# rpp0/gr-lora

Measured on AMD Instinct MI355X. Metric: IQ Msamples/s demodulated, higher is better.
Workload: dtype f32

## Files before the change

### gr_lora_amd/build.py

```python
from __future__ import annotations

import os
import shutil
import subprocess

_HERE = os.path.dirname(os.path.abspath(__file__))
CSRC = os.path.join(_HERE, "csrc")
LIB = os.path.join(_HERE, "liblora_hip.so")
SOURCES = ["lora_kernels.hip", "lora_runtime.cpp", "lora_channelizer.hip", "lora_filterbank.hip", "lora_iq_unpack.hip", "lora_gateway.cpp", "lora_frame_check.cpp", "lora_tx.hip"]
DEPS = SOURCES + ["lora_device.h", "lora_stitch.hpp", "lora_walker2.inc.hip", "lora_walker3.inc.hip", "lora_team_demod.inc.hip", "lora_wave_demod.inc.hip", "lora_wave_decim.inc.hip", "lora_detect.inc.hip", "lora_strict_sync.inc.hip", "lora_strict_resolve_lds.inc", "whitening_data.inc", "lora_mux_dev.h", "lora_iq.h", "lora_frame_check.h",
                  os.path.join("..", "..", "include", "lora_hip.h"), os.path.join("..", "..", "include", "lora_hip_channelizer.h"),
                  os.path.join("..", "..", "include", "lora_hip_filterbank.h"), os.path.join("..", "..", "include", "lora_hip_gateway.h"),
                  os.path.join("..", "..", "include", "lora_hip_tx.h")]


CODEGEN_FLAGS = ["-mllvm", "-greedy-reverse-local-assignment"]


def hipcc_path() -> str:
    return shutil.which("hipcc") or "/opt/rocm/bin/hipcc"


def stale() -> bool:
    if not os.path.exists(LIB):
        return True
    t = os.path.getmtime(LIB)
    return any(os.path.getmtime(os.path.join(CSRC, d)) > t for d in DEPS)


def build_library(force: bool = False, verbose: bool = False) -> str:
    if not force and not stale():
        return LIB
    cmd = [hipcc_path(), "--offload-arch=gfx950", "-O3", "-std=c++17", "-fPIC", "-shared", "-x", "hip",
           "-Wall", "-Wno-unused-function"] + CODEGEN_FLAGS + os.environ.get("LORA_HIP_EXTRA_FLAGS", "").split() + ["-I", CSRC, "-o", LIB] + [os.path.join(CSRC, s) for s in SOURCES]
    if verbose:
        cmd.insert(1, "-Rpass-analysis=kernel-resource-usage")
    subprocess.check_call(cmd)
    return LIB


if __name__ == "__main__":
    import sys
    print(build_library(force=True, verbose="-v" in sys.argv))
# ... 1 lines not shown
```

### gr_lora_amd/csrc/lora_device.h

```cpp
#pragma once
#include <stdint.h>

#if !defined(__HIPCC__) && !defined(HIP_INCLUDE_HIP_HIP_RUNTIME_H)
struct float2 { float x, y; };
#endif

namespace lora_hip {

constexpr int kWG = 256;
constexpr int kMaxBinsPerThread = 16;
constexpr int kMaxFrame = 3 + 255 + 2;
constexpr int kMaxCodewords = 640;

enum DecState : int32_t { kDetect = 0, kSync, kFindSfd, kPause, kDecodeHeader, kDecodePayload, kStop };

enum AttemptStatus : uint32_t {
    kAttemptNone = 0,
    kAttemptFrame = 1,
    kAttemptLostSync = 2,
    kAttemptOutOfData = 3,
    kAttemptAtHeader = 4,
    kAttemptAtSfd = 5,
    kAttemptHeaderOnly = 6
};
struct SkippedPayload {
    uint8_t  phdr[3];
    uint8_t  n_left;
    uint8_t  left[8];
    int32_t  payload_symbols;
};
constexpr float kSfdIllVar = 1.0f / 4096.0f;
constexpr int kMaxSfdRec = 12;

struct DevParams {
    uint32_t sf, nbins, nbins_hdr, sps, decim, log_nbins, delay_after_sync;
    uint32_t implicit, reduced_rate, enable_fine_sync, demod_mode;
    uint32_t ctor_cr, ctor_crc;
    uint32_t use_fast;
// ... 69 lines not shown
    int64_t  tail_final_pos;
    uint32_t tail_valid, tail_first_rec, tail_n_attempts, tail_final_cr, tail_npush, tail_stop_reason, tail_pad, tail_rsv;
    float    tail_push_tail[4];
    uint32_t ctl[4];
    uint32_t dbg[6];
};

struct StepRec {
    int32_t  state, consumed;
    int64_t  pos;
    int32_t  bin, fine;
    float    value;
    uint32_t stream;
    uint32_t cycles;
    uint32_t pad;
};

struct LaunchCfg {
    const float2 *iq;
    const Job *jobs;
    JobResult *results;
    AttemptRec *recs;
    uint32_t recs_per_job;
    float *scratch;
    StepRec *trace;
    uint32_t trace_cap;
    uint32_t n_jobs;
    uint32_t *balance;
    uint32_t skip_payload;
};
constexpr uint32_t kBalanceCus = 2048;
constexpr uint32_t kBalanceWords = 3u * kBalanceCus;

struct EnvStream {
    uint64_t off;
    uint32_t first_block;
    uint32_t n_blocks;
};
int launch_envelope(const float2 *iq, const EnvStream *streams , uint32_t n_streams, uint32_t sps,
                    float *d_E, unsigned long long *d_bitmap , void *stream);

int launch_walker(const DevParams &p, const LaunchCfg &c, void *stream);
const char *walker_kernel_name(const DevParams &p);
struct DemodAlt { int32_t *shift; uint32_t *bins; int32_t *fine; int64_t max_start; };
int launch_demod_symbols(const DevParams &p, const float2 *iq, const int64_t *d_offsets, uint32_t n,
                         int demod, uint32_t *d_bins, int32_t *d_fine, float *scratch, void *stream, const DemodAlt *alt = nullptr);
int launch_detect_windows(const DevParams &p, const float2 *iq, const int64_t *d_offsets, uint32_t n, void *d_out , void *stream);
constexpr int kPayloadHyp = 4;
struct PayloadDesc {
    uint32_t n_walk;
    uint32_t n_hyp;
    int32_t  hyp_shift[kPayloadHyp];
    int32_t  hyp_base[kPayloadHyp];
    uint32_t hyp_from[kPayloadHyp];
    uint32_t hyp_to[kPayloadHyp];
    int64_t  room;
    SkippedPayload sk;
};
enum PayloadWalk : uint32_t { kWalkComplete = 0, kWalkOutOfData = 1, kWalkNeedShift = 2 };
struct PayloadOut {
    uint32_t result;
    uint32_t at;
    int32_t  shift;
    uint32_t frame_len;
    uint8_t  frame[kMaxFrame + 4];
};
int launch_payload_chain(const DevParams &p, const uint32_t *d_bins, const int32_t *d_fine, const DemodAlt &alt, const PayloadDesc *descs, PayloadOut *outs, uint32_t n_packets, void *stream);
bool walker_has_skip_variant(const DevParams &p);
int launch_ref_ifreq(const float2 *x, uint32_t n, float *d_arg, float *d_ifreq, void *stream);
int launch_cfo(const DevParams &p, const float2 *iq, const int64_t *d_offsets, uint32_t n, int mode, float *d_out, void *stream);
bool walker3_covers(uint32_t sf);
uint32_t w3_tw_entries(uint32_t sf);
void build_w3_tables(uint32_t sf, float2 *tw, float2 *ctab );
// ... 13 lines not shown
```

### gr_lora_amd/csrc/lora_kernels.hip

```cpp

#include <hip/hip_runtime.h>
#include <math.h>
#include <stdio.h>
#include <atomic>
#include <cstdlib>
#include <stdint.h>
#include <type_traits>

#include "lora_device.h"
#include "whitening_data.inc"

namespace lora_hip {

__constant__ unsigned char c_whiten_cr56[LORA_WHITEN_CR56_LEN];
__constant__ unsigned char c_whiten_cr78[LORA_WHITEN_CR78_LEN];
__constant__ unsigned char c_h84_decode[256];
static std::atomic<bool> g_consts_ready[16];

static unsigned char h_hamming_encode(unsigned v)
{
    const unsigned b0 = v & 1u, b1 = (v >> 1) & 1u, b2 = (v >> 2) & 1u, b3 = (v >> 3) & 1u;
    const unsigned p1 = b1 ^ b2 ^ b3, p2 = b0 ^ b1 ^ b2, p3 = b0 ^ b1 ^ b3, p4 = b0 ^ b2 ^ b3;
    return (unsigned char)(p1 | (b0 << 1) | (b1 << 2) | (b2 << 3) | (p2 << 4) | (b3 << 5) | (p3 << 6) | (p4 << 7));
}
// ... 773 lines not shown

        if (end_step(st_in, consumed, step_bin, fine, step_val, t_start)) break;
    }

    if (in_attempt && n_att < C.recs_per_job && t0) {
        AttemptRec &r = recs[n_att];
        r.status = (stop_reason == 3u) ? kAttemptAtHeader : kAttemptOutOfData;
        r.start_pos = att_start; r.trig_pos = att_trig; r.hdr_pos = att_hdr; r.end_pos = pos;
        r.npush = npush;
        for (int i = 0; i < 4; i++) r.push_tail[i] = push_tail[i];
        r.cr_prev = att_cr_prev; r.hdr_ambig = att_ambig; r.n_symbols = n_sym; r.frame_len = 0; r.n_sfd = 0;
    }
    if (t0) {
        JobResult &jr = C.results[jid];
        jr.final_pos = in_attempt ? att_start : pos;
        jr.n_attempts = n_att + (in_attempt ? 1u : 0u);
        jr.final_cr = cr;
        jr.npush = in_attempt ? 0u : npush;
        for (int i = 0; i < 4; i++) jr.push_tail[i] = push_tail[i];
        jr.stop_reason = stop_reason;
        jr.n_steps = n_steps < C.trace_cap ? n_steps : C.trace_cap;
        jr.pad = in_attempt ? 1u : 0u;
        for (int i = 0; i < 6; i++) { jr.cyc[i] = 0; jr.rounds[i] = 0; }
        jr.tail_valid = 0;
    }
}

__global__ __launch_bounds__(kWG) void walker_kernel(DevParams P, LaunchCfg C) { walker_body<2>(P, C); }
__global__ __launch_bounds__(kWG) void walker_kernel_f1(DevParams P, LaunchCfg C) { walker_body<1>(P, C); }
__global__ __launch_bounds__(kWG) void walker_kernel_f0(DevParams P, LaunchCfg C) { walker_body<0>(P, C); }

#include "lora_wave_demod.inc.hip"
#include "lora_wave_decim.inc.hip"
#include "lora_walker2.inc.hip"
#include "lora_walker3.inc.hip"
#include "lora_team_demod.inc.hip"

__global__ __launch_bounds__(kWG) void demod_symbols_kernel(DevParams P, const float2 *iq, const int64_t *offsets,
                                                            uint32_t n, int demod, uint32_t *bins, float *scratch)
{
    extern __shared__ __attribute__((aligned(16))) unsigned char smem[];
    float2 *work = reinterpret_cast<float2 *>(smem);
    float *fl = reinterpret_cast<float *>(smem);
    Shared &sh = *reinterpret_cast<Shared *>(smem + P.lds_work_bytes);
    for (uint32_t s = blockIdx.x; s < n; s += gridDim.x) {
        const float2 *x = iq + offsets[s];
        uint32_t b;
        if (demod == 0) {
            float *f1 = P.ifreq_in_lds_1 ? fl : scratch + (size_t)blockIdx.x * 2u * P.sps;
            compute_ifreq(x, P.sps, f1);
            b = gradient_idx_from_ifreq(P, f1, sh.red);
        } else {
            b = get_shift_fft(P, x, work, sh.red);
        }
        if (threadIdx.x == 0) bins[s] = b;
        __syncthreads();
    }
}

constexpr uint32_t kPayloadMaxWalk = 1024;
__global__ __launch_bounds__(64) void payload_chain_kernel(DevParams P, const uint32_t *__restrict__ bins, const int32_t *__restrict__ fine, DemodAlt alt,
                                                           const PayloadDesc *__restrict__ descs, PayloadOut *__restrict__ outs, uint32_t n_packets)
{
    __shared__ Shared sh;
    __shared__ PayloadDesc d;
    __shared__ uint32_t src[kPayloadMaxWalk];
// ... 231 lines not shown
    if (ensure_constants() != 0) return -1;
    if (c.skip_payload && !walker_has_skip_variant(p)) return -1;
    const WalkerKernel k = pick_for_launch(p, c.n_jobs, c.skip_payload != 0);
    if (k.lds > 64u * 1024u) {
        static thread_local const void *last_fn = nullptr;
        static thread_local uint32_t last_lds = 0;
        static thread_local int last_dev = -1;
        int dev = 0;
        (void)hipGetDevice(&dev);
        if (last_fn != (const void *)k.fn || last_lds < k.lds || last_dev != dev) {
            if (hipFuncSetAttribute((const void *)k.fn, hipFuncAttributeMaxDynamicSharedMemorySize, (int)k.lds) != hipSuccess) return -1;
            last_fn = (const void *)k.fn; last_lds = k.lds; last_dev = dev;
        }
    }
    hipLaunchKernelGGL(k.fn, dim3(c.n_jobs), dim3(k.threads), k.lds, (hipStream_t)stream, p, c);
    return hipGetLastError() == hipSuccess ? 0 : -1;
}

uint32_t walker_resident_slots(const DevParams &p)
{
    return slots_of(pick_walker(p, w3_has_half(p) && w3_half_policy() != 0));
}
uint32_t walker_resident_slots_full(const DevParams &p)
{
    if (use_fast_kernel(p) || use_fast_decim(p)) {
        int dev = 0, cus = 0;
        if (hipGetDevice(&dev) != hipSuccess || hipDeviceGetAttribute(&cus, hipDeviceAttributeMultiprocessorCount, dev) != hipSuccess || cus <= 0) cus = 256;
        const uint32_t s = slots_of(pick_walker(p));
        return s > (uint32_t)cus ? (uint32_t)cus : 0u;
    }
    return (w3_has_half(p) && w3_half_policy() < 0) ? slots_of(pick_walker(p, false)) : 0u;
}

constexpr int kEnvLines = 4;
constexpr uint32_t kEnvTableMax = 64;
struct EnvTable { EnvStream s[kEnvTableMax]; };

__global__ __launch_bounds__(256) void envelope_kernel(const float2 *iq, EnvTable T, uint32_t sps, float *E)
{
    const EnvStream s = T.s[blockIdx.y];
    const uint32_t b = (blockIdx.x * 256u + threadIdx.x) >> 3, li = threadIdx.x & 7u;
    const bool live = b < s.n_blocks;
    float e = 0.0f;
    if (live) {
        const float4 *x = reinterpret_cast<const float4 *>(iq + ((s.off + (uint64_t)b * sps) & ~1ull)) + li;
        const uint32_t stride = sps >> 3;
        float4 v[kEnvLines];
#pragma unroll
        for (int l = 0; l < kEnvLines; l++) v[l] = x[(uint32_t)l * stride];
#pragma unroll
        for (int l = 0; l < kEnvLines; l++) e += v[l].x * v[l].x + v[l].y * v[l].y + v[l].z * v[l].z + v[l].w * v[l].w;
    }
    e += __shfl_xor(e, 1); e += __shfl_xor(e, 2); e += __shfl_xor(e, 4);
    if (live && li == 0) E[s.first_block + b] = e;
}

constexpr int kEnvReach = 8;

__global__ __launch_bounds__(256) void edges_kernel(EnvTable T, const float *E, unsigned long long *bitmap)
{
    const EnvStream s = T.s[blockIdx.y];
    const uint32_t b = blockIdx.x * 256u + threadIdx.x;
    bool edge = false;
    if (b >= 1u && b < s.n_blocks) {
        const float *Es = E + s.first_block;
        float m1 = 0.0f, m0 = 0.0f;
#pragma unroll
        for (int d = -kEnvReach - 1; d <= kEnvReach; d++) {
            const int64_t q = (int64_t)b + d;
            const float v = (q >= 0 && q < (int64_t)s.n_blocks) ? Es[q] : 0.0f;
            if (d >= -kEnvReach) m1 = fmaxf(m1, v);
            if (d < kEnvReach) m0 = fmaxf(m0, v);
        }
        edge = Es[b] < 0.5f * m1 && !(Es[b - 1u] < 0.5f * m0);
    }
    const unsigned long long word = __ballot(edge);
    if ((threadIdx.x & 63u) == 0u && b < s.n_blocks) bitmap[(s.first_block + b) >> 6] = word;
}

int launch_envelope(const float2 *iq, const EnvStream *streams , uint32_t n_streams, uint32_t sps, float *d_E,
                    unsigned long long *d_bitmap, void *stream)
{
    if (n_streams == 0 || sps < 128u) return -1;
    for (uint32_t s0 = 0; s0 < n_streams; s0 += kEnvTableMax) {
        const uint32_t n = n_streams - s0 < kEnvTableMax ? n_streams - s0 : kEnvTableMax;
        EnvTable T{};
        uint32_t most = 0;
        for (uint32_t i = 0; i < n; i++) { T.s[i] = streams[s0 + i]; most = most > T.s[i].n_blocks ? most : T.s[i].n_blocks; }
        if (most == 0) continue;
        hipLaunchKernelGGL(envelope_kernel, dim3((most + 31u) / 32u, n), dim3(256), 0, (hipStream_t)stream, iq, T, sps, d_E);
        hipLaunchKernelGGL(edges_kernel, dim3((most + 255u) / 256u, n), dim3(256), 0, (hipStream_t)stream, T, (const float *)d_E, d_bitmap);
    }
    return hipGetLastError() == hipSuccess ? 0 : -1;
}

__global__ __launch_bounds__(256) void cfo_kernel(DevParams P, const float2 *__restrict__ iq, const int64_t *__restrict__ offsets, uint32_t n, int mode,
                                                  float *__restrict__ out)
{
    __shared__ double dred[256];
    const uint32_t sps = P.sps;
    for (uint32_t s = blockIdx.x; s < n; s += gridDim.x) {
        const float2 *x = iq + offsets[s];
        auto dechirped = [&](uint32_t i) {
            const float2 a = x[i], b = P.down[i];
            return make_float2(a.x * b.x - a.y * b.y, a.x * b.y + a.y * b.x);
        };
        if (mode == 0) {
            if (threadIdx.x == 0) out[s] = (float)((double)ifreq_pair(dechirped(256u), dechirped(257u)) / (2.0 * M_PI) * (double)P.samples_per_second);
            continue;
        }
        double acc = 0.0;
        for (uint32_t i = threadIdx.x; i + 1u < sps; i += blockDim.x) acc += (double)ifreq_pair(dechirped(i), dechirped(i + 1u));
        dred[threadIdx.x] = acc;
        __syncthreads();
        for (uint32_t h = 128u; h >= 1u; h >>= 1) {
            if (threadIdx.x < h) dred[threadIdx.x] += dred[threadIdx.x + h];
            __syncthreads();
        }
        if (threadIdx.x == 0) out[s] = (float)(dred[0] / (double)(sps - 1u) / (2.0 * M_PI) * (double)P.samples_per_second);
        __syncthreads();
    }
}

__global__ void ref_ifreq_kernel(const float2 *__restrict__ x, uint32_t n, float *__restrict__ arg_out, float *__restrict__ ifreq_out)
// ... 144 lines not shown
```

### gr_lora_amd/csrc/lora_runtime.cpp

```cpp

#include <hip/hip_runtime.h>

#include <algorithm>
#include <cmath>
#include <cstddef>
#include <cstdarg>
#include <cstdio>
#include <cstdlib>
#include <cstring>
#include <chrono>
#include <deque>
#include <new>
#include <string>
#include <vector>

#include "../../include/lora_hip.h"
#include "lora_device.h"
#include "lora_stitch.hpp"
#include "lora_mux_dev.h"
#include "lora_iq.h"

using namespace lora_hip;

namespace {
// ... 100 lines not shown
    size_t n_up_ifreq_v = 0;
    DevBuf<Job> d_jobs;
    DevBuf<JobResult> d_results;
    DevBuf<AttemptRec> d_recs;
    DevBuf<float> d_scratch;
    DevBuf<StepRec> d_trace;
    DevBuf<float2> d_staging;
    DevBuf<int64_t> d_offsets;
    DevBuf<uint32_t> d_bins;
    RunOut run_out[2];
    std::vector<JobResult> h_results;
    std::vector<AttemptRec> h_recs;
    std::vector<StepRec> h_trace;
    hipEvent_t ev0 = nullptr, ev1 = nullptr, ev_done = nullptr;
    hipEvent_t ev_pre0 = nullptr, ev_pre1 = nullptr, ev_dep = nullptr;
    hipStream_t pre_stream = nullptr;
    struct Pending { uint32_t nj = 0, recs_per_job = 0, eager = 0, trace_cap = 0; bool direct = true, open = false; hipStream_t st = nullptr;
                     std::chrono::steady_clock::time_point hp0, hp1; } pending;
    PassCtx pass;
    std::vector<StreamDesc> pass_streams;
    const float2 *pass_iq = nullptr;
    hipStream_t pass_st = nullptr;
    bool pass_open = false, iq_ready = false;
    bool pre_issued = false;
    const float2 *pre_iq = nullptr;
    uint64_t pre_sig = 0;
    uint32_t pre_ns = 0;
    std::chrono::steady_clock::time_point pre_hq0;
    FrameQueue frames;
    PinnedBuf<Job> p_jobs;
    PinnedBuf<JobResult> p_res;
    PinnedBuf<AttemptRec> p_recs;
    DevBuf<uint32_t> d_balance;
    DevBuf<float> d_env_E;
    DevBuf<unsigned long long> d_env_buf;
    PinnedBuf<EnvStream> p_env_streams;
    PinnedBuf<unsigned long long> p_env_buf;
    float envelope_ms = 0.0f;
    std::vector<lora_hip_step_t> trace;
    lora_hip_timing_t timing{};
    std::string err;
    ChunkPipe pipe;
    struct HostFeed {
        PinnedBuf<float2> stage[2];
        hipEvent_t stage_ev[2] = {nullptr, nullptr};
        bool stage_busy[2] = {false, false};
        int stage_i = 0;
        DevBuf<uint32_t> d_raw;
        std::vector<std::pair<uintptr_t, uintptr_t>> pinned;
        std::vector<std::pair<uintptr_t, uintptr_t>> refused;
    } feed;
    const char *last_kernel = nullptr;
    uint32_t last_kernel_jobs = 0;
    uint32_t resident_slots = 0;
    uint32_t resident_slots_alt = ~0u;
    uint32_t eager_recs = 4;
    uint32_t last_plan_burst = 0, last_plan_segments = 0;
    int decoupled_policy = -1;
    bool launch_skip = false;
    uint32_t dec_backoff = 0;
    uint32_t last_payload_packets = 0, last_payload_rerun = 0, last_payload_symbols = 0, last_payload_moved = 0, last_payload_rounds = 0;
    float last_payload_ms = 0.0f;
    PinnedBuf<int64_t> p_pay_off;
    PinnedBuf<PayloadDesc> p_pay_desc;
    PinnedBuf<PayloadOut> p_pay_out;
    DevBuf<int32_t> d_fine, d_alt_shift, d_alt_fine;
    DevBuf<uint32_t> d_alt_bins;
// ... 219 lines not shown
        HIP_TRY(h, h->d_recs.reserve((size_t)nj * recs_per_job));
    }
    const bool need_scratch = !h->P.ifreq_in_lds_2;
    if (need_scratch) HIP_TRY(h, h->d_scratch.reserve((size_t)nj * 2u * h->P.sps));
    if (trace_cap) HIP_TRY(h, h->d_trace.reserve((size_t)nj * trace_cap));
    static const bool direct = getenv("LORA_HIP_STAGED") == nullptr;
    const uint32_t eager = direct ? recs_per_job : std::min(std::max(h->eager_recs, 2u), recs_per_job);
    HIP_TRY(h, h->p_jobs.reserve(nj));
    HIP_TRY(h, h->p_res.reserve(nj));
    HIP_TRY(h, h->p_recs.reserve((size_t)nj * eager));
    std::memcpy(h->p_jobs.p, jobs.data(), nj * sizeof(Job));
    if (!direct) HIP_TRY(h, hipMemcpyAsync(h->d_jobs.p, h->p_jobs.p, nj * sizeof(Job), hipMemcpyHostToDevice, st));
    LaunchCfg c{};
    c.iq = d_iq; c.recs_per_job = recs_per_job;
    c.jobs = direct ? h->p_jobs.p : h->d_jobs.p; c.results = direct ? h->p_res.p : h->d_results.p; c.recs = direct ? h->p_recs.p : h->d_recs.p;
    c.scratch = need_scratch ? h->d_scratch.p : nullptr;
    c.trace = trace_cap ? h->d_trace.p : nullptr; c.trace_cap = trace_cap; c.n_jobs = nj;
    static const bool no_balance = getenv("LORA_HIP_NO_BALANCE") != nullptr;
    if (!h->d_balance.p && !no_balance) {
        HIP_TRY(h, h->d_balance.reserve(kBalanceWords));
        HIP_TRY(h, hipMemsetAsync(h->d_balance.p, 0, kBalanceWords * sizeof(uint32_t), st));
    }
    c.balance = no_balance ? nullptr : h->d_balance.p;
    c.skip_payload = h->launch_skip ? 1u : 0u;
    HIP_TRY(h, hipEventRecord(h->ev0, st));
    if (nj >= h->last_kernel_jobs) { h->last_kernel = walker_kernel_name_for(h->P, nj, h->launch_skip); h->last_kernel_jobs = nj; }
    if (launch_walker(h->P, c, st) != 0) return fail(h, LORA_HIP_ERR_HIP, "walker launch failed: %s", hipGetErrorString(hipGetLastError()));
    HIP_TRY(h, hipEventRecord(h->ev1, st));
    if (!direct) {
        HIP_TRY(h, hipMemcpyAsync(h->p_res.p, h->d_results.p, nj * sizeof(JobResult), hipMemcpyDeviceToHost, st));
        HIP_TRY(h, hipMemcpy2DAsync(h->p_recs.p, eager * sizeof(AttemptRec), h->d_recs.p, recs_per_job * sizeof(AttemptRec), eager * sizeof(AttemptRec), nj,
                                    hipMemcpyDeviceToHost, st));
    }
    HIP_TRY(h, hipEventRecord(h->ev_done, st));
    h->pending.eager = eager; h->pending.direct = direct; h->pending.open = true;
    h->pending.hp1 = std::chrono::steady_clock::now();
    return LORA_HIP_OK;
}

lora_hip_status run_jobs_end(lora_hip_decoder *h, RunOut &out)
{
    if (!h->pending.open) return LORA_HIP_OK;
    h->pending.open = false;
    const uint32_t nj = h->pending.nj, recs_per_job = h->pending.recs_per_job, eager = h->pending.eager, trace_cap = h->pending.trace_cap;
    const hipStream_t st = h->pending.st;
    const auto hp0 = h->pending.hp0, hp1 = h->pending.hp1;
    const Job *jobs = h->p_jobs.p;
    HIP_TRY(h, hipEventSynchronize(h->ev_done));
    const auto hp2 = std::chrono::steady_clock::now();
    std::memcpy(out.res.data(), h->p_res.p, nj * sizeof(JobResult));
    static const bool dbg_stats = getenv("LORA_HIP_DEBUG") != nullptr;
    if (dbg_stats && h->P.use_fast) {
        double cyc[6] = {0}, rnd[6] = {0};
        for (uint32_t j = 0; j < nj; j++) for (int i = 0; i < 6; i++) { cyc[i] += 64.0 * out.res[j].cyc[i]; rnd[i] += out.res[j].rounds[i]; }
        fprintf(stderr, "[lora_hip] per-job avg kcycles (rounds): DETECT %.0f (%.1f) SYNC %.0f (%.1f) SFD %.0f (%.1f) PAUSE %.0f (%.1f) HDR %.0f (%.1f) PAYLOAD %.0f (%.1f)\n",
                cyc[0] / nj / 1e3, rnd[0] / nj, cyc[1] / nj / 1e3, rnd[1] / nj, cyc[2] / nj / 1e3, rnd[2] / nj, cyc[3] / nj / 1e3, rnd[3] / nj, cyc[4] / nj / 1e3, rnd[4] / nj, cyc[5] / nj / 1e3, rnd[5] / nj);
        {
            double na = 0, nt = 0, ntv = 0; uint32_t sr[4] = {0, 0, 0, 0}, tsr[4] = {0, 0, 0, 0}, tpad = 0;
            for (uint32_t j = 0; j < nj; j++) {
                const JobResult &r = out.res[j];
                na += r.n_attempts; sr[r.stop_reason & 3u]++;
                if (r.tail_valid) { ntv++; nt += r.tail_n_attempts; tsr[r.tail_stop_reason & 3u]++; tpad += r.tail_pad; }
            }
            fprintf(stderr, "[lora_hip] attempts/job %.2f, stop reasons %u/%u/%u/%u; tails %.0f (attempts/tail %.2f, stop reasons %u/%u/%u/%u, pending %u)\n", na / nj, sr[0], sr[1],
                    sr[2], sr[3], ntv, ntv ? nt / ntv : 0.0, tsr[0], tsr[1], tsr[2], tsr[3], tpad);
        }
        double ctl[4] = {0};
        for (uint32_t j = 0; j < nj; j++) for (int i = 0; i < 4; i++) ctl[i] += 64.0 * out.res[j].ctl[i];
        fprintf(stderr, "[lora_hip] control per job, kcycles: copy-in %.0f loop %.0f plan %.0f copy-out %.0f (walker3: demodulation %.0f, replay %.0f of the decode rounds; with LORA_W3_REPLAY_STATS=2 copy-in and symbol loop in the 3rd / 4th figure)\n", ctl[0] / nj / 1e3, ctl[1] / nj / 1e3, ctl[2] / nj / 1e3, ctl[3] / nj / 1e3, ctl[0] / nj / 1e3, ctl[1] / nj / 1e3);
        std::vector<double> tot(nj);
        for (uint32_t j = 0; j < nj; j++) { double t = 0; for (int i = 0; i < 6; i++) t += 64.0 * out.res[j].cyc[i]; tot[j] = t; }
        std::sort(tot.begin(), tot.end());
        double mean = 0; for (double t : tot) mean += t; mean /= nj;
        fprintf(stderr, "[lora_hip] job kcycles over %u jobs: min %.0f p50 %.0f p90 %.0f max %.0f mean %.0f\n", nj, tot[0] / 1e3, tot[nj / 2] / 1e3,
                tot[(size_t)(nj * 0.9)] / 1e3, tot[nj - 1] / 1e3, mean / 1e3);
    }
    if (const char *tl = getenv("LORA_HIP_JOB_TIMELINE")) {
        if (FILE *f = fopen(tl, "a")) {
            fprintf(f, "# launch of %u jobs: job hw_id xcc_id t_start t_end(100MHz) cyc[6] x64 start scan_limit n_att\n", nj);
            for (uint32_t j = 0; j < nj; j++) {
                const JobResult &r = out.res[j];
// ... 62 lines not shown
lora_hip_status run_jobs(lora_hip_decoder *h, const float2 *d_iq, const std::vector<Job> &jobs, uint32_t recs_per_job, uint32_t trace_cap,
                         hipStream_t st, RunOut &out)
{
    const lora_hip_status s = run_jobs_begin(h, d_iq, jobs, recs_per_job, trace_cap, st, out);
    return s == LORA_HIP_OK ? run_jobs_end(h, out) : s;
}

void append_trace(lora_hip_decoder *h, const RunOut &out, uint32_t job_index, uint32_t trace_cap, int64_t abs_base)
{
    const JobResult &jr = out.res[job_index];
    for (uint32_t i = 0; i < jr.n_steps; i++) {
        const StepRec &s = h->h_trace[(size_t)job_index * trace_cap + i];
        lora_hip_step_t o;
        o.state = s.state; o.consumed = s.consumed; o.pos = abs_base + s.pos; o.bin = s.bin; o.fine = s.fine;
        o.value = s.value; o.stream = s.stream; o.cycles = s.cycles; o.reserved = 0;
        h->trace.push_back(o);
    }
}

uint64_t streams_signature(const std::vector<StreamDesc> &streams)
{
    uint64_t x = 1469598103934665603ull;
    for (const StreamDesc &sd : streams)
        for (uint64_t v : {sd.off, sd.len}) { x ^= v; x *= 1099511628211ull; }
    return x ^ streams.size();
}

lora_hip_status quiet_edges_enqueue(lora_hip_decoder *h, const float2 *d_iq, const std::vector<StreamDesc> &streams, hipStream_t st)
{
    const uint32_t sps = h->P.sps, ns = (uint32_t)streams.size();
    h->pre_issued = false;
    h->pre_hq0 = std::chrono::steady_clock::now();
    HIP_TRY(h, h->p_env_streams.reserve(ns));
    uint64_t nb = 0;
    for (uint32_t i = 0; i < ns; i++) {
        const uint64_t n = streams[i].len / sps;
        nb = (nb + 63u) & ~63ull;
        if (n == 0 || nb + n > 0xffffffffull) return LORA_HIP_ERR_ARG;
        h->p_env_streams.p[i] = EnvStream{streams[i].off, (uint32_t)nb, (uint32_t)n};
        nb += n;
    }
    const size_t words = (size_t)((nb + 63u) / 64u);
    HIP_TRY(h, h->d_env_E.reserve(nb));
    HIP_TRY(h, h->d_env_buf.reserve(words));
    HIP_TRY(h, h->p_env_buf.reserve(words));
    const hipStream_t ps = h->pre_stream;
    if (!h->iq_ready) {
        HIP_TRY(h, hipEventRecord(h->ev_dep, st));
        HIP_TRY(h, hipStreamWaitEvent(ps, h->ev_dep, 0));
    }
    static const bool dbg = getenv("LORA_HIP_DEBUG") != nullptr;
    if (dbg) HIP_TRY(h, hipEventRecord(h->ev_pre0, ps));
    static const bool direct = getenv("LORA_HIP_STAGED") == nullptr;
    if (launch_envelope(d_iq, h->p_env_streams.p, ns, sps, h->d_env_E.p, direct ? h->p_env_buf.p : h->d_env_buf.p, ps) != 0)
        return fail(h, LORA_HIP_ERR_HIP, "envelope launch failed: %s", hipGetErrorString(hipGetLastError()));
    if (dbg) HIP_TRY(h, hipEventRecord(h->ev_pre1, ps));
    if (!direct) HIP_TRY(h, hipMemcpyAsync(h->p_env_buf.p, h->d_env_buf.p, words * 8u, hipMemcpyDeviceToHost, ps));
    h->pre_issued = true; h->pre_iq = d_iq; h->pre_sig = streams_signature(streams); h->pre_ns = ns;
    return LORA_HIP_OK;
}

lora_hip_status quiet_edges_collect(lora_hip_decoder *h, std::vector<std::vector<int64_t>> &edges)
{
    if (!h->pre_issued) return LORA_HIP_ERR_ARG;
    h->pre_issued = false;
    const uint32_t sps = h->P.sps, ns = h->pre_ns;
    static const bool dbg = getenv("LORA_HIP_DEBUG") != nullptr;
    const auto hq0 = h->pre_hq0, hq1 = std::chrono::steady_clock::now();
    HIP_TRY(h, hipStreamSynchronize(h->pre_stream));
    const auto hq2 = std::chrono::steady_clock::now();
    if (dbg) { float ms = 0; if (hipEventElapsedTime(&ms, h->ev_pre0, h->ev_pre1) == hipSuccess) h->envelope_ms = ms; }
    edges.resize(ns);
    uint32_t n_found = 0;
    const unsigned long long *bm = h->p_env_buf.p;
    for (uint32_t i = 0; i < ns; i++) {
        std::vector<int64_t> &e = edges[i];
        e.clear();
        const uint64_t b0 = h->p_env_streams.p[i].first_block, b1 = b0 + h->p_env_streams.p[i].n_blocks;
        for (uint64_t w = b0 / 64u; w * 64u < b1; w++) {
            unsigned long long bits = bm[w];
            while (bits) {
                const uint64_t b = w * 64u + (uint64_t)__builtin_ctzll(bits);
                bits &= bits - 1ull;
                if (b >= b0 && b < b1) e.push_back((int64_t)(b - b0) * (int64_t)sps);
            }
        }
        n_found += (uint32_t)e.size();
// ... 190 lines not shown
        if (h->decoupled_policy < 0 && packets >= 4u && 4u * (rerun + moved) > packets) h->dec_backoff = 32;
        static const bool dbg = getenv("LORA_HIP_DEBUG") != nullptr;
        if (dbg) fprintf(stderr, "[lora_hip] payload pass: %u packets, %u symbol reads in %u round(s), %.3f ms; %u packet(s) ended off the zero-drift grid (their jobs split there), %u handed to the complete kernels\n",
                         packets, h->last_payload_symbols, h->last_payload_rounds, h->last_payload_ms, moved, rerun);
    }
    RunOut &run_out(int which) { return h->run_out[which & 1]; }
    bool quiet_edges(const std::vector<StreamDesc> &streams, std::vector<std::vector<int64_t>> &edges)
    {
        return ::quiet_edges(h, d_iq, streams, st, edges) == LORA_HIP_OK;
    }
    int run_jobs(const std::vector<Job> &jobs, uint32_t rpj, uint32_t trace_cap, RunOut &out)
    {
        return ::run_jobs(h, d_iq, jobs, rpj, trace_cap, st, out) == LORA_HIP_OK ? 0 : -1;
    }
    int run_jobs_begin(const std::vector<Job> &jobs, uint32_t rpj, uint32_t trace_cap, RunOut &out)
    {
        return ::run_jobs_begin(h, d_iq, jobs, rpj, trace_cap, st, out) == LORA_HIP_OK ? 0 : -1;
    }
    int run_jobs_end(RunOut &out) { return ::run_jobs_end(h, out) == LORA_HIP_OK ? 0 : -1; }
    void publish(const AttemptRec &r, StreamDesc &sd) { ::publish(h, r, sd); }
    void append_trace(const RunOut &out, uint32_t job, uint32_t cap, int64_t base) { ::append_trace(h, out, job, cap, base); }
    void count_jobs(uint32_t n) { h->timing.jobs += n; h->last_kernel_jobs = 0; if (h->dec_backoff) h->dec_backoff--; }
    void count_probes(uint32_t n) { h->timing.probes += n; }
    void count_slow_path() { h->timing.slow_path_relaunches++; }
    void count_repair()
    {
        static const bool dbg = getenv("LORA_HIP_DEBUG") != nullptr;
        if (dbg) fprintf(stderr, "[lora_hip] cut repaired from the true header (no serial walk)\n");
    }
    void note_plan(bool burst_aware, size_t n_segs)
    {
        h->last_plan_burst = burst_aware ? 1u : 0u; h->last_plan_segments = (uint32_t)n_segs;
        static const bool dbg = getenv("LORA_HIP_DEBUG") != nullptr;
        if (dbg) fprintf(stderr, "[lora_hip] segment plan: %s, %zu segments (envelope kernels %.3f ms)\n", burst_aware ? "burst-aware" : "fixed grid", n_segs, burst_aware ? h->envelope_ms : 0.0f);
    }
    double walker_ms() const { return h->timing.walker_ms; }
};

lora_hip_status scheduler_failed(lora_hip_decoder *h)
{
    h->pending.open = false;
    return h->err.empty() ? fail(h, LORA_HIP_ERR_INTERNAL, "scheduler failed") : LORA_HIP_ERR_HIP;
}

lora_hip_status pass_begin(lora_hip_decoder *h, const float2 *d_iq, hipStream_t st, bool iq_ready)
{
    h->pass_iq = d_iq; h->pass_st = st;
    h->iq_ready = iq_ready;
    h->err.clear();
    DeviceEnv env{h, d_iq, st};
    const int rc = lora_hip::decode_begin(env, h->pass_streams, h->pass);
    h->iq_ready = false;
    if (rc != 0) return scheduler_failed(h);
    h->pass_open = true;
    return LORA_HIP_OK;
}

lora_hip_status pass_end(lora_hip_decoder *h)
{
    h->pass_open = false;
    h->err.clear();
    DeviceEnv env{h, h->pass_iq, h->pass_st};
    return lora_hip::decode_end(env, h->pass_streams, h->pass) == 0 ? LORA_HIP_OK : scheduler_failed(h);
}


void pipe_init(lora_hip_decoder *h, uint32_t n_channels, size_t batch)
// ... 49 lines not shown
        if (tail > p.tailcap) {
            const size_t ncap = std::max(2u * p.tailcap, tail + (size_t)h->P.sps), nregion = ncap + p.batch;
            HIP_TRY(h, hipStreamSynchronize(p.copy_st));
            HIP_TRY(h, hipStreamSynchronize(p.comp_st));
            for (int i = 0; i < 2; i++) {
                DevBuf<float2> nb;
                HIP_TRY(h, nb.reserve(p.ch.size() * nregion));
                for (size_t q = 0; q < p.ch.size(); q++)
                    HIP_TRY(h, hipMemcpyAsync(nb.p + q * nregion + (ncap - p.tailcap), p.dbuf[i].p + q * p.region, p.region * sizeof(float2), hipMemcpyDeviceToDevice, p.comp_st));
                HIP_TRY(h, hipStreamSynchronize(p.comp_st));
                std::swap(p.dbuf[i], nb);
                nb.release();
            }
            for (StreamDesc &x : h->pass_streams) x.off = (x.off / p.region) * nregion + (x.off % p.region) + (ncap - p.tailcap);
            p.tailcap = ncap; p.region = nregion;
        }
        if (tail) {
            HIP_TRY(h, hipMemcpyAsync(p.dbuf[p.cur].p + (size_t)sd.id * p.region + p.tailcap - tail, p.dbuf[p.cur ^ 1].p + sd.off + keep_from, tail * sizeof(float2),
                                      hipMemcpyDeviceToDevice, p.comp_st));
            any_tail = true;
        }
        c.tail_len = tail;
    }
    if (any_tail) {
        HIP_TRY(h, hipEventRecord(p.tail_ev, p.comp_st));
        HIP_TRY(h, hipStreamWaitEvent(p.copy_st, p.tail_ev, 0));
    }
    return LORA_HIP_OK;
}

lora_hip_status pipe_collect_if_done(lora_hip_decoder *h)
{
    lora_hip_status s = LORA_HIP_OK;
    if (h->pipe.inflight && h->pending.open && hipEventQuery(h->ev_done) == hipSuccess) s = pipe_collect(h);
    (void)hipGetLastError();
    return s;
}

lora_hip_status pipe_rotate(lora_hip_decoder *h, bool by_latency)
{
    ChunkPipe &p = h->pipe;
    HIP_TRY(h, hipEventRecord(p.up_ev, p.copy_st));
    lora_hip_status s = pipe_collect(h);
    if (s != LORA_HIP_OK) return s;
    std::vector<StreamDesc> &sds = h->pass_streams;
    sds.clear();
    for (uint32_t c = 0; c < p.ch.size(); c++) {
        ChunkPipe::Chan &C = p.ch[c];
        const size_t len = C.tail_len + C.fill;
        if (len < 2u * (size_t)h->P.sps) continue;
        StreamDesc sd{};
        sd.off = (uint64_t)c * p.region + p.tailcap - C.tail_len; sd.len = len; sd.id = c;
        sd.cr_in = C.cr; sd.pwr = C.pwr; sd.abs_base = C.host_base;
        sds.push_back(sd);
    }
    if (sds.empty()) return LORA_HIP_OK;
    HIP_TRY(h, hipStreamWaitEvent(p.comp_st, p.up_ev, 0));
    h->timing = lora_hip_timing_t{};
    for (const StreamDesc &sd : sds) h->timing.items += sd.len;
    s = pass_begin(h, p.dbuf[p.cur].p, p.comp_st, false);
    if (s != LORA_HIP_OK) return s;
    p.inflight = true;
    p.passes++; p.passes_by_latency += by_latency ? 1u : 0u;
    p.cur ^= 1;
    p.have_first = false;
    for (uint32_t c = 0; c < p.ch.size(); c++) {
        ChunkPipe::Chan &C = p.ch[c];
// ... 55 lines not shown
                             hipEventCreateWithFlags(&h->ev_dep, hipEventDisableTiming) != hipSuccess ||
                             hipStreamCreateWithFlags(&h->pre_stream, hipStreamNonBlocking) != hipSuccess ||
                             hipStreamCreateWithFlags(&h->pay_stream, hipStreamNonBlocking) != hipSuccess || hipEventCreate(&h->ev_pay0) != hipSuccess ||
                             hipEventCreate(&h->ev_pay1) != hipSuccess || hipEventCreate(&h->ev_pay_done) != hipSuccess))
        s = LORA_HIP_ERR_HIP;
    if (s != LORA_HIP_OK) { lora_hip_destroy(h); return s; }
    pipe_init(h, 1, cfg->batch_items ? cfg->batch_items : std::max<size_t>(1u << 20, 64ull * h->P.sps));
    *out = h;
    return LORA_HIP_OK;
}

void lora_hip_destroy(lora_hip_decoder_t *h)
{
    if (!h) return;
    (void)hipSetDevice(h->device);
    if (h->pipe.comp_st) { (void)hipStreamSynchronize(h->pipe.copy_st); (void)hipStreamSynchronize(h->pipe.comp_st); }
    if (h->d_down) (void)hipFree(h->d_down);
    if (h->d_twN) (void)hipFree(h->d_twN);
    if (h->d_tws) (void)hipFree(h->d_tws);
    if (h->d_wave_tabs) (void)hipFree(h->d_wave_tabs);
    if (h->d_w3_tw) (void)hipFree(h->d_w3_tw);
    if (h->d_team_tabs) (void)hipFree(h->d_team_tabs);
    if (h->d_w3_ctab) (void)hipFree(h->d_w3_ctab);
    if (h->d_up_ifreq) (void)hipFree(h->d_up_ifreq);
    if (h->d_down_ifreq) (void)hipFree(h->d_down_ifreq);
    if (h->d_up_ifreq_v) (void)hipFree(h->d_up_ifreq_v);
    h->p_pay_off.release(); h->p_pay_desc.release(); h->p_pay_out.release(); h->d_fine.release(); h->d_alt_shift.release(); h->d_alt_bins.release(); h->d_alt_fine.release();
    h->d_jobs.release(); h->d_results.release(); h->d_recs.release(); h->d_scratch.release();
    h->d_trace.release(); h->d_staging.release(); h->d_offsets.release(); h->d_bins.release();
    for (auto &r : h->feed.pinned) (void)hipHostUnregister((void *)r.first);
    for (int i = 0; i < 2; i++) { h->pipe.dbuf[i].release(); h->feed.stage[i].release(); }
    h->feed.d_raw.release();
    h->p_jobs.release(); h->p_res.release(); h->p_recs.release();
    h->d_balance.release(); h->d_env_E.release(); h->d_env_buf.release(); h->p_env_streams.release(); h->p_env_buf.release();
    for (hipEvent_t e : {h->ev0, h->ev1, h->ev_done, h->ev_pre0, h->ev_pre1, h->ev_dep, h->ev_pay0, h->ev_pay1, h->ev_pay_done, h->pipe.up_ev, h->pipe.tail_ev,
                         h->feed.stage_ev[0], h->feed.stage_ev[1]})
        if (e) (void)hipEventDestroy(e);
    for (hipStream_t st : {h->pre_stream, h->pay_stream, h->pipe.copy_st, h->pipe.comp_st})
        if (st) (void)hipStreamDestroy(st);
    delete h;
}

lora_hip_status lora_hip_get_table(const lora_hip_decoder_t *h, int which, float *buf, size_t cap_floats, size_t *n_floats)
{
    if (!h) return LORA_HIP_ERR_ARG;
    const size_t sps = h->P.sps;
    const void *src = nullptr;
    size_t n = 0;
    bool on_device = true;
    switch (which) {
    case 0: src = h->d_down; n = 2 * sps; break;
    case 1: src = h->h_up.data(); n = 2 * sps; on_device = false; break;
    case 2: src = h->d_down_ifreq; n = sps; break;
    case 3: src = h->d_up_ifreq; n = sps; break;
    case 4: src = h->d_up_ifreq_v; n = h->n_up_ifreq_v; break;
    default: return LORA_HIP_ERR_ARG;
    }
    if (n_floats) *n_floats = n;
    if (!buf) return LORA_HIP_OK;
    if (cap_floats < n || !src) return LORA_HIP_ERR_ARG;
    if (!on_device) { memcpy(buf, src, n * sizeof(float)); return LORA_HIP_OK; }
    if (hipSetDevice(h->device) != hipSuccess || hipMemcpy(buf, src, n * sizeof(float), hipMemcpyDeviceToHost) != hipSuccess) return LORA_HIP_ERR_HIP;
    return LORA_HIP_OK;
}

lora_hip_status lora_hip_get_geometry(const lora_hip_decoder_t *h, uint32_t *sps, uint32_t *bins, uint32_t *decim)
{
// ... 816 lines not shown
```

Before: 265,800.

## Fuse envelope and edge kernels into one tiled prepass with LDS halo

Merges the envelope energy kernel and the edge-detection kernel into a single prepass kernel that computes per-block energies for a tile plus halo into shared memory, then detects edges and writes the bitmap directly. This removes the intermediate global energy buffer, one kernel launch and its global round trip, at the cost of recomputing halo energies at tile boundaries. Separately, in direct mode the runtime now waits on an existing event instead of recording an extra ev_done event.

```diff
diff --git a/gr_lora_amd/build.py b/gr_lora_amd/build.py
--- a/gr_lora_amd/build.py
+++ b/gr_lora_amd/build.py
@@ -8,7 +8,7 @@
 CSRC = os.path.join(_HERE, "csrc")
 LIB = os.path.join(_HERE, "liblora_hip.so")
 SOURCES = ["lora_kernels.hip", "lora_runtime.cpp", "lora_channelizer.hip", "lora_filterbank.hip", "lora_iq_unpack.hip", "lora_gateway.cpp", "lora_frame_check.cpp", "lora_tx.hip"]
-DEPS = SOURCES + ["lora_device.h", "lora_stitch.hpp", "lora_walker2.inc.hip", "lora_walker3.inc.hip", "lora_team_demod.inc.hip", "lora_wave_demod.inc.hip", "lora_wave_decim.inc.hip", "lora_detect.inc.hip", "lora_strict_sync.inc.hip", "lora_strict_resolve_lds.inc", "whitening_data.inc", "lora_mux_dev.h", "lora_iq.h", "lora_frame_check.h",
+DEPS = SOURCES + ["lora_device.h", "lora_prepass_tiles.h", "lora_prepass.inc.hip", "lora_stitch.hpp", "lora_walker2.inc.hip", "lora_walker3.inc.hip", "lora_team_demod.inc.hip", "lora_wave_demod.inc.hip", "lora_wave_decim.inc.hip", "lora_detect.inc.hip", "lora_strict_sync.inc.hip", "lora_strict_resolve_lds.inc", "whitening_data.inc", "lora_mux_dev.h", "lora_iq.h", "lora_frame_check.h",
                   os.path.join("..", "..", "include", "lora_hip.h"), os.path.join("..", "..", "include", "lora_hip_channelizer.h"),
                   os.path.join("..", "..", "include", "lora_hip_filterbank.h"), os.path.join("..", "..", "include", "lora_hip_gateway.h"),
                   os.path.join("..", "..", "include", "lora_hip_tx.h")]
diff --git a/gr_lora_amd/csrc/lora_device.h b/gr_lora_amd/csrc/lora_device.h
--- a/gr_lora_amd/csrc/lora_device.h
+++ b/gr_lora_amd/csrc/lora_device.h
@@ -4,6 +4,7 @@
 #if !defined(__HIPCC__) && !defined(HIP_INCLUDE_HIP_HIP_RUNTIME_H)
 struct float2 { float x, y; };
 #endif
+#include "lora_prepass_tiles.h"
 
 namespace lora_hip {
 
@@ -139,13 +140,8 @@
 constexpr uint32_t kBalanceCus = 2048;
 constexpr uint32_t kBalanceWords = 3u * kBalanceCus;
 
-struct EnvStream {
-    uint64_t off;
-    uint32_t first_block;
-    uint32_t n_blocks;
-};
 int launch_envelope(const float2 *iq, const EnvStream *streams , uint32_t n_streams, uint32_t sps,
-                    float *d_E, unsigned long long *d_bitmap , void *stream);
+                    unsigned long long *d_bitmap , void *stream);
 
 int launch_walker(const DevParams &p, const LaunchCfg &c, void *stream);
 const char *walker_kernel_name(const DevParams &p);
diff --git a/gr_lora_amd/csrc/lora_kernels.hip b/gr_lora_amd/csrc/lora_kernels.hip
--- a/gr_lora_amd/csrc/lora_kernels.hip
+++ b/gr_lora_amd/csrc/lora_kernels.hip
@@ -829,6 +829,7 @@
 
 #include "lora_wave_demod.inc.hip"
 #include "lora_wave_decim.inc.hip"
+#include "lora_prepass.inc.hip"
 #include "lora_walker2.inc.hip"
 #include "lora_walker3.inc.hip"
 #include "lora_team_demod.inc.hip"
@@ -1126,53 +1127,7 @@
     return (w3_has_half(p) && w3_half_policy() < 0) ? slots_of(pick_walker(p, false)) : 0u;
 }
 
-constexpr int kEnvLines = 4;
-constexpr uint32_t kEnvTableMax = 64;
-struct EnvTable { EnvStream s[kEnvTableMax]; };
-
-__global__ __launch_bounds__(256) void envelope_kernel(const float2 *iq, EnvTable T, uint32_t sps, float *E)
-{
-    const EnvStream s = T.s[blockIdx.y];
-    const uint32_t b = (blockIdx.x * 256u + threadIdx.x) >> 3, li = threadIdx.x & 7u;
-    const bool live = b < s.n_blocks;
-    float e = 0.0f;
-    if (live) {
-        const float4 *x = reinterpret_cast<const float4 *>(iq + ((s.off + (uint64_t)b * sps) & ~1ull)) + li;
-        const uint32_t stride = sps >> 3;
-        float4 v[kEnvLines];
-#pragma unroll
-        for (int l = 0; l < kEnvLines; l++) v[l] = x[(uint32_t)l * stride];
-#pragma unroll
-        for (int l = 0; l < kEnvLines; l++) e += v[l].x * v[l].x + v[l].y * v[l].y + v[l].z * v[l].z + v[l].w * v[l].w;
-    }
-    e += __shfl_xor(e, 1); e += __shfl_xor(e, 2); e += __shfl_xor(e, 4);
-    if (live && li == 0) E[s.first_block + b] = e;
-}
-
-constexpr int kEnvReach = 8;
-
-__global__ __launch_bounds__(256) void edges_kernel(EnvTable T, const float *E, unsigned long long *bitmap)
-{
-    const EnvStream s = T.s[blockIdx.y];
-    const uint32_t b = blockIdx.x * 256u + threadIdx.x;
-    bool edge = false;
-    if (b >= 1u && b < s.n_blocks) {
-        const float *Es = E + s.first_block;
-        float m1 = 0.0f, m0 = 0.0f;
-#pragma unroll
-        for (int d = -kEnvReach - 1; d <= kEnvReach; d++) {
-            const int64_t q = (int64_t)b + d;
-            const float v = (q >= 0 && q < (int64_t)s.n_blocks) ? Es[q] : 0.0f;
-            if (d >= -kEnvReach) m1 = fmaxf(m1, v);
-            if (d < kEnvReach) m0 = fmaxf(m0, v);
-        }
-        edge = Es[b] < 0.5f * m1 && !(Es[b - 1u] < 0.5f * m0);
-    }
-    const unsigned long long word = __ballot(edge);
-    if ((threadIdx.x & 63u) == 0u && b < s.n_blocks) bitmap[(s.first_block + b) >> 6] = word;
-}
-
-int launch_envelope(const float2 *iq, const EnvStream *streams , uint32_t n_streams, uint32_t sps, float *d_E,
+int launch_envelope(const float2 *iq, const EnvStream *streams , uint32_t n_streams, uint32_t sps,
                     unsigned long long *d_bitmap, void *stream)
 {
     if (n_streams == 0 || sps < 128u) return -1;
@@ -1182,8 +1137,7 @@
         uint32_t most = 0;
         for (uint32_t i = 0; i < n; i++) { T.s[i] = streams[s0 + i]; most = most > T.s[i].n_blocks ? most : T.s[i].n_blocks; }
         if (most == 0) continue;
-        hipLaunchKernelGGL(envelope_kernel, dim3((most + 31u) / 32u, n), dim3(256), 0, (hipStream_t)stream, iq, T, sps, d_E);
-        hipLaunchKernelGGL(edges_kernel, dim3((most + 255u) / 256u, n), dim3(256), 0, (hipStream_t)stream, T, (const float *)d_E, d_bitmap);
+        hipLaunchKernelGGL(prepass_kernel, dim3((most + kEnvTile - 1u) / kEnvTile, n), dim3(256), 0, (hipStream_t)stream, iq, T, sps, d_bitmap);
     }
     return hipGetLastError() == hipSuccess ? 0 : -1;
 }
diff --git a/gr_lora_amd/csrc/lora_prepass.inc.hip b/gr_lora_amd/csrc/lora_prepass.inc.hip
--- /dev/null
+++ b/gr_lora_amd/csrc/lora_prepass.inc.hip
@@ -0,0 +1,65 @@
+constexpr int kEnvLines = 4;
+constexpr int kEnvBatch = 3;
+
+__device__ __forceinline__ void env_tile(const float2 *iq, const EnvStream s, uint32_t t0, uint32_t sps, float *Es, unsigned long long *bitmap,
+                                         uint32_t tid, uint32_t nthreads)
+{
+    const uint32_t li = tid & 7u, groups = nthreads >> 3;
+    const uint32_t stride = sps >> 3;
+    uint32_t lo, hi;
+    env_tile_span(s, t0, lo, hi);
+    for (uint32_t g0 = tid >> 3; g0 < kEnvTileE + (tid >> 3); g0 += groups * kEnvBatch) {
+        float4 v[kEnvBatch][kEnvLines];
+        bool live[kEnvBatch];
+#pragma unroll
+        for (int k = 0; k < kEnvBatch; k++) {
+            const int64_t b = (int64_t)t0 - (int64_t)kEnvHalo + (int64_t)(g0 + (uint32_t)k * groups);
+            live[k] = g0 + (uint32_t)k * groups < kEnvTileE && b >= (int64_t)lo && b < (int64_t)hi;
+            if (live[k]) {
+                const float4 *x = reinterpret_cast<const float4 *>(iq + ((s.off + (uint64_t)b * sps) & ~1ull)) + li;
+#pragma unroll
+                for (int l = 0; l < kEnvLines; l++) v[k][l] = x[(uint32_t)l * stride];
+            }
+        }
+#pragma unroll
+        for (int k = 0; k < kEnvBatch; k++) {
+            float e = 0.0f;
+            if (live[k]) {
+#pragma unroll
+                for (int l = 0; l < kEnvLines; l++) e += v[k][l].x * v[k][l].x + v[k][l].y * v[k][l].y + v[k][l].z * v[k][l].z + v[k][l].w * v[k][l].w;
+            }
+            e += __shfl_xor(e, 1); e += __shfl_xor(e, 2); e += __shfl_xor(e, 4);
+            const uint32_t g = g0 + (uint32_t)k * groups;
+            if (li == 0u && g < kEnvTileE) Es[g] = e;
+        }
+    }
+    __syncthreads();
+    for (uint32_t i = tid; i < kEnvTile; i += nthreads) {
+        const uint32_t b = t0 + i;
+        const float *Eb = Es + kEnvHalo + i;
+        bool edge = false;
+        if (b >= 1u && b < s.n_blocks) {
+            float m1 = 0.0f, m0 = 0.0f;
+#pragma unroll
+            for (int d = -kEnvReach - 1; d <= kEnvReach; d++) {
+                const float v = Eb[d];
+                if (d >= -kEnvReach) m1 = fmaxf(m1, v);
+                if (d < kEnvReach) m0 = fmaxf(m0, v);
+            }
+            edge = Eb[0] < 0.5f * m1 && !(Eb[-1] < 0.5f * m0);
+        }
+        const unsigned long long word = __ballot(edge);
+        if ((i & 63u) == 0u && b < s.n_blocks) bitmap[(s.first_block + b) >> 6] = word;
+    }
+}
+
+constexpr uint32_t kEnvTableMax = 64;
+struct EnvTable { EnvStream s[kEnvTableMax]; };
+
+__global__ __launch_bounds__(256) void prepass_kernel(const float2 *iq, EnvTable T, uint32_t sps, unsigned long long *bitmap)
+{
+    __shared__ float Es[kEnvTileE];
+    const EnvStream s = T.s[blockIdx.y];
+    if (blockIdx.x * kEnvTile >= s.n_blocks) return;
+    env_tile(iq, s, blockIdx.x * kEnvTile, sps, Es, bitmap, threadIdx.x, 256u);
+}
diff --git a/gr_lora_amd/csrc/lora_prepass_tiles.h b/gr_lora_amd/csrc/lora_prepass_tiles.h
--- /dev/null
+++ b/gr_lora_amd/csrc/lora_prepass_tiles.h
@@ -0,0 +1,46 @@
+#pragma once
+#include <stddef.h>
+#include <stdint.h>
+
+#if defined(__HIPCC__)
+#define LORA_ENV_HD __host__ __device__
+#else
+#define LORA_ENV_HD
+#endif
+
+namespace lora_hip {
+
+struct EnvStream {
+    uint64_t off;
+    uint32_t first_block;
+    uint32_t n_blocks;
+};
+
+constexpr int kEnvReach = 8;
+constexpr uint32_t kEnvTile = 256;
+constexpr uint32_t kEnvHalo = (uint32_t)kEnvReach + 1u;
+constexpr uint32_t kEnvTileE = kEnvTile + 2u * kEnvHalo;
+
+LORA_ENV_HD inline void env_tile_span(const EnvStream &s, uint32_t t0, uint32_t &lo, uint32_t &hi)
+{
+    lo = t0 > kEnvHalo ? t0 - kEnvHalo : 0u;
+    const uint64_t end = (uint64_t)t0 + kEnvTile + kEnvHalo;
+    hi = end < s.n_blocks ? (uint32_t)end : s.n_blocks;
+    if (lo > hi) lo = hi;
+}
+
+inline uint64_t env_layout(const uint64_t *off, const uint64_t *len, uint32_t n_streams, uint32_t sps, EnvStream *out)
+{
+    uint64_t nb = 0;
+    if (sps == 0u) return 0;
+    for (uint32_t i = 0; i < n_streams; i++) {
+        const uint64_t n = len[i] / sps;
+        nb = (nb + 63u) & ~63ull;
+        if (n == 0 || nb + n > 0xffffffffull) return 0;
+        out[i] = EnvStream{off[i], (uint32_t)nb, (uint32_t)n};
+        nb += n;
+    }
+    return nb;
+}
+
+}
diff --git a/gr_lora_amd/csrc/lora_runtime.cpp b/gr_lora_amd/csrc/lora_runtime.cpp
--- a/gr_lora_amd/csrc/lora_runtime.cpp
+++ b/gr_lora_amd/csrc/lora_runtime.cpp
@@ -156,7 +156,6 @@
     PinnedBuf<JobResult> p_res;
     PinnedBuf<AttemptRec> p_recs;
     DevBuf<uint32_t> d_balance;
-    DevBuf<float> d_env_E;
     DevBuf<unsigned long long> d_env_buf;
     PinnedBuf<EnvStream> p_env_streams;
     PinnedBuf<unsigned long long> p_env_buf;
@@ -442,7 +441,7 @@
         HIP_TRY(h, hipMemcpy2DAsync(h->p_recs.p, eager * sizeof(AttemptRec), h->d_recs.p, recs_per_job * sizeof(AttemptRec), eager * sizeof(AttemptRec), nj,
                                     hipMemcpyDeviceToHost, st));
     }
-    HIP_TRY(h, hipEventRecord(h->ev_done, st));
+    if (!direct) HIP_TRY(h, hipEventRecord(h->ev_done, st));
     h->pending.eager = eager; h->pending.direct = direct; h->pending.open = true;
     h->pending.hp1 = std::chrono::steady_clock::now();
     return LORA_HIP_OK;
@@ -456,7 +455,7 @@
     const hipStream_t st = h->pending.st;
     const auto hp0 = h->pending.hp0, hp1 = h->pending.hp1;
     const Job *jobs = h->p_jobs.p;
-    HIP_TRY(h, hipEventSynchronize(h->ev_done));
+    HIP_TRY(h, hipEventSynchronize(h->pending.direct ? h->ev1 : h->ev_done));
     const auto hp2 = std::chrono::steady_clock::now();
     std::memcpy(out.res.data(), h->p_res.p, nj * sizeof(JobResult));
     static const bool dbg_stats = getenv("LORA_HIP_DEBUG") != nullptr;
@@ -585,17 +584,13 @@
     h->pre_issued = false;
     h->pre_hq0 = std::chrono::steady_clock::now();
     HIP_TRY(h, h->p_env_streams.reserve(ns));
-    uint64_t nb = 0;
-    for (uint32_t i = 0; i < ns; i++) {
-        const uint64_t n = streams[i].len / sps;
-        nb = (nb + 63u) & ~63ull;
-        if (n == 0 || nb + n > 0xffffffffull) return LORA_HIP_ERR_ARG;
-        h->p_env_streams.p[i] = EnvStream{streams[i].off, (uint32_t)nb, (uint32_t)n};
-        nb += n;
-    }
+    std::vector<uint64_t> off(ns), len(ns);
+    for (uint32_t i = 0; i < ns; i++) { off[i] = streams[i].off; len[i] = streams[i].len; }
+    const uint64_t nb = env_layout(off.data(), len.data(), ns, sps, h->p_env_streams.p);
+    if (nb == 0) return LORA_HIP_ERR_ARG;
     const size_t words = (size_t)((nb + 63u) / 64u);
-    HIP_TRY(h, h->d_env_E.reserve(nb));
-    HIP_TRY(h, h->d_env_buf.reserve(words));
+    static const bool direct = getenv("LORA_HIP_STAGED") == nullptr;
+    if (!direct) HIP_TRY(h, h->d_env_buf.reserve(words));
     HIP_TRY(h, h->p_env_buf.reserve(words));
     const hipStream_t ps = h->pre_stream;
     if (!h->iq_ready) {
@@ -604,8 +599,7 @@
     }
     static const bool dbg = getenv("LORA_HIP_DEBUG") != nullptr;
     if (dbg) HIP_TRY(h, hipEventRecord(h->ev_pre0, ps));
-    static const bool direct = getenv("LORA_HIP_STAGED") == nullptr;
-    if (launch_envelope(d_iq, h->p_env_streams.p, ns, sps, h->d_env_E.p, direct ? h->p_env_buf.p : h->d_env_buf.p, ps) != 0)
+    if (launch_envelope(d_iq, h->p_env_streams.p, ns, sps, direct ? h->p_env_buf.p : h->d_env_buf.p, ps) != 0)
         return fail(h, LORA_HIP_ERR_HIP, "envelope launch failed: %s", hipGetErrorString(hipGetLastError()));
     if (dbg) HIP_TRY(h, hipEventRecord(h->ev_pre1, ps));
     if (!direct) HIP_TRY(h, hipMemcpyAsync(h->p_env_buf.p, h->d_env_buf.p, words * 8u, hipMemcpyDeviceToHost, ps));
@@ -862,7 +856,7 @@
     {
         h->last_plan_burst = burst_aware ? 1u : 0u; h->last_plan_segments = (uint32_t)n_segs;
         static const bool dbg = getenv("LORA_HIP_DEBUG") != nullptr;
-        if (dbg) fprintf(stderr, "[lora_hip] segment plan: %s, %zu segments (envelope kernels %.3f ms)\n", burst_aware ? "burst-aware" : "fixed grid", n_segs, burst_aware ? h->envelope_ms : 0.0f);
+        if (dbg) fprintf(stderr, "[lora_hip] segment plan: %s, %zu segments (envelope kernel %.3f ms)\n", burst_aware ? "burst-aware" : "fixed grid", n_segs, burst_aware ? h->envelope_ms : 0.0f);
     }
     double walker_ms() const { return h->timing.walker_ms; }
 };
@@ -978,7 +972,7 @@
 lora_hip_status pipe_collect_if_done(lora_hip_decoder *h)
 {
     lora_hip_status s = LORA_HIP_OK;
-    if (h->pipe.inflight && h->pending.open && hipEventQuery(h->ev_done) == hipSuccess) s = pipe_collect(h);
+    if (h->pipe.inflight && h->pending.open && hipEventQuery(h->pending.direct ? h->ev1 : h->ev_done) == hipSuccess) s = pipe_collect(h);
     (void)hipGetLastError();
     return s;
 }
@@ -1100,7 +1094,7 @@
     for (int i = 0; i < 2; i++) { h->pipe.dbuf[i].release(); h->feed.stage[i].release(); }
     h->feed.d_raw.release();
     h->p_jobs.release(); h->p_res.release(); h->p_recs.release();
-    h->d_balance.release(); h->d_env_E.release(); h->d_env_buf.release(); h->p_env_streams.release(); h->p_env_buf.release();
+    h->d_balance.release(); h->d_env_buf.release(); h->p_env_streams.release(); h->p_env_buf.release();
     for (hipEvent_t e : {h->ev0, h->ev1, h->ev_done, h->ev_pre0, h->ev_pre1, h->ev_dep, h->ev_pay0, h->ev_pay1, h->ev_pay_done, h->pipe.up_ev, h->pipe.tail_ev,
                          h->feed.stage_ev[0], h->feed.stage_ev[1]})
         if (e) (void)hipEventDestroy(e);
```

Result: no change. 269,800, median of 6 (+1.5%).
